# Mouafak-Khaled/Flow-Q-Learning

Hardware: AMD Instinct MI355X
Metric: FQL grad-steps/sec (whole node) over 16-α population, cube-single-v0 (higher is better)
Workload: dtype f32

## Files before the change

### flow-q-learning_amd/csrc/kernels.h

```cpp
#pragma once
#include <hip/hip_runtime.h>
#include <stdint.h>

namespace fq {

struct TRef {
    float* p;
    long long ss;
    long long sy;
};

inline TRef tref(float* p, long long ss, long long sy = 0) { return TRef{p, ss, sy}; }

enum GemmLayout { LAYOUT_FWD = 0, LAYOUT_DX = 1, LAYOUT_DW = 2 };
enum GemmEpi { EPI_STORE = 0, EPI_BIAS = 1, EPI_BIAS_GELU2 = 2, EPI_BIAS_GELU = 3, EPI_ADAM = 4 };

struct GemmArgs {
    TRef A, B, C, C2, bias;
    int M, N, K;
    int lda, ldb, ldc;
    int ny, nz;
    const int* slots;
    unsigned long long* probe;
};
void launch_gemm(int layout, int epi, int tile, const GemmArgs& a, hipStream_t s);
void launch_gemm_euler_hidden(const GemmArgs& a, hipStream_t s);
void launch_gemm_variant(int layout, int epi, int tile, int variant, const GemmArgs& a, hipStream_t s);
constexpr int GEMM_GROUP_MAX = 8;
constexpr int HP_COUNT = 3;
enum { HP_LR = 0, HP_DISCOUNT = 1, HP_TAU = 2 };
struct Chunk { long long off; int len; int leaf; };
struct AdamArgs {
    const float* p_in;
    float* p_out;
    float *g, *m, *v;
    float* target;
    long long P, PT;
    long long net_off;
    const Chunk* chunks;
    const int* ids;
    int n_chunks, chunk_base;
    float* stats;
    int n_total_chunks;
    const int* count;
    const float* hparams;
    int nz;
    const int* slots;
};
struct AdamEpi {
    const float* p_in;
    float *p_out, *m, *v, *target, *wt_out;
    long long P, PT, PTT;
    long long ens, wt_sy;
    long long w_off[GEMM_GROUP_MAX];
    long long wt_off[GEMM_GROUP_MAX];
    int stat_base[GEMM_GROUP_MAX];
    float* stats;
    int n_total_chunks;
    const int* count;
    const float* hparams;
    int mode;
    int nt;
    AdamArgs small;
    int small_blocks;
};
struct GemmGroupArgs {
    GemmArgs g[GEMM_GROUP_MAX];
    int first[GEMM_GROUP_MAX + 1];
    int ng;
    AdamEpi adam;
// ... 49 lines not shown
    long long w_off[EF_MAX_LAYERS + 1], b_off[EF_MAX_LAYERS + 1];
    long long g_off[EF_MAX_LAYERS], be_off[EF_MAX_LAYERS];
    const float* x0;
    long long x0_ss;
    int ld_x, K0, L, M;
    float* U[EF_MAX_LAYERS];
    float* G[EF_MAX_LAYERS];
    float* MU[EF_MAX_LAYERS];
    float* RS[EF_MAX_LAYERS];
    long long s_ss, s_sy, st_ss, st_sy;
    int ld_s, st_lo, st_hi;
    int g_hi;
    HeadArgs head;
    int ny, nz;
    const int* slots;
};
bool stream_fwd_supported(int H, int L, int K0, int nout, int M);
void launch_stream_fwd(int head_mode, bool ln, const StreamArgs& a, hipStream_t s);

struct SplitSync {
    unsigned long long* xch;
    unsigned* cnt;
    unsigned* gen;
    unsigned* err;
};
struct SplitFwdArgs {
    StreamArgs s;
    TRef aflow;
    int D, A, S, first;
    float steps_f;
// ... 303 lines not shown
```

### flow-q-learning_amd/csrc/kernels.hip

```cpp
#include "kernels.h"

#include <hip/hip_runtime.h>
#include <math.h>

#include <type_traits>

#if defined(__HIP_DEVICE_COMPILE__) && !defined(__gfx950__)
#error "fqlpop kernels target gfx950 (MI355X) only: the s_waitcnt immediates use the gfx9 encoding"
#endif


namespace fq {

typedef float f32x16 __attribute__((ext_vector_type(16)));
typedef float f32x4 __attribute__((ext_vector_type(4)));

#define DEV __device__ __forceinline__

DEV float* at(TRef t, int slot, int y = 0) {
    return t.p + (long long)slot * t.ss + (long long)y * t.sy;
}

constexpr float kSqrt2OverPi = 0.7978845608028654f;

// ... 106 lines not shown
    const int slot = a.slots[z];
    const Chunk ck = a.chunks[ci];
    const long long base = (long long)slot * a.P + a.net_off + ck.off;
    const float t = (float)(a.count[slot] + 1);
    const float bc1 = 1.0f - powf(0.9f, t), bc2 = 1.0f - powf(0.999f, t);
    float mx = -INFINITY, mn = INFINITY, ss = 0.f;
    const float* hp = a.hparams + (long long)slot * HP_COUNT;
    const float lr = hp[HP_LR], tau = hp[HP_TAU];
    const bool hasT = a.target != nullptr;
    if (NT == 256 || threadIdx.x < 256) {
        const float* __restrict__ Pin = a.p_in + base;
        float* __restrict__ P = a.p_out + base;
        const float* __restrict__ G = a.g + base;
        float* __restrict__ Mm = a.m + base;
        float* __restrict__ V = a.v + base;
        float* __restrict__ T = hasT ? a.target + (long long)slot * a.PT + ck.off : nullptr;
        auto one = [&](float g, float& p, float& m, float& v, float& tp) {
            adam_moments(g, m, v);
            if (hasT) tp = ema_target(p, tp, tau);
            p = adam_step_ieee(p, m, v, bc1, bc2, lr);
            mx = fmaxf(mx, g);
            mn = fminf(mn, g);
            ss = fmaf(g, g, ss);
        };
        if ((ck.len & 3) == 0) {
            for (int i = threadIdx.x * 4; i < ck.len; i += 1024) {
                const float4 g4 = *reinterpret_cast<const float4*>(G + i);
                float4 p4 = *reinterpret_cast<const float4*>(Pin + i);
                float4 m4 = *reinterpret_cast<float4*>(Mm + i);
                float4 v4 = *reinterpret_cast<float4*>(V + i);
                float4 t4 = make_float4(0.f, 0.f, 0.f, 0.f);
                if (hasT) t4 = *reinterpret_cast<float4*>(T + i);
                one(g4.x, p4.x, m4.x, v4.x, t4.x);
                one(g4.y, p4.y, m4.y, v4.y, t4.y);
                one(g4.z, p4.z, m4.z, v4.z, t4.z);
                one(g4.w, p4.w, m4.w, v4.w, t4.w);
                *reinterpret_cast<float4*>(P + i) = p4;
                *reinterpret_cast<float4*>(Mm + i) = m4;
                *reinterpret_cast<float4*>(V + i) = v4;
                if (hasT) *reinterpret_cast<float4*>(T + i) = t4;
            }
        } else {
            for (int i = threadIdx.x; i < ck.len; i += 256) {
                const float gv = G[i];
                float p = Pin[i], m = Mm[i], v = V[i], tv = hasT ? T[i] : 0.f;
                one(gv, p, m, v, tv);
                P[i] = p;
                Mm[i] = m;
                V[i] = v;
                if (hasT) T[i] = tv;
            }
        }
    }
    __shared__ float red[3 * 8];
    float st3[3] = {mx, mn, ss};
    block_reduce_n<3>(st3, {1, 2, 0}, red);
    mx = st3[0];
    mn = st3[1];
    ss = st3[2];
    if (threadIdx.x == 0) {
        float* st = a.stats + ((long long)slot * a.n_total_chunks + ci) * 3;
        st[0] = mx;
        st[1] = mn;
        st[2] = ss;
    }
// ... 98 lines not shown
    else __builtin_amdgcn_raw_buffer_store_b128(w, r, off_b, 0, 0);
}

constexpr int ADAM_U = 2;
struct AdamPre {
    float4 p[ADAM_U], m[ADAM_U], v[ADAM_U], t[ADAM_U];
};
template <int BM, int BN>
DEV void adam_issue0(const AdamEpi& e, int gi, const GemmArgs& g, int slot, int y, int i0, int j0, AdamPre& pre) {
    constexpr int TPR = BN / 4, RPI = 256 / TPR;
    const int gM = uni(g.M), ldc = uni(g.ldc), tid = threadIdx.x;
    const long long pb = uni64((long long)slot * e.P + e.w_off[gi] + (long long)y * e.ens);
    const long long nleaf = (long long)gM * ldc;
    const rsrc_t rP = make_rsrc(e.p_in + pb, nleaf);
    const rsrc_t rM = make_rsrc(e.m + pb, nleaf), rV = make_rsrc(e.v + pb, nleaf);
    const bool hasT = e.target != nullptr;
    const rsrc_t rT = make_rsrc(uniptr(hasT ? e.target + (long long)slot * e.PT + e.w_off[gi] + (long long)y * e.ens
                                            : e.m + pb), nleaf);
    const int cj = (tid % TPR) * 4, ri = tid / TPR;
#pragma unroll
    for (int u = 0; u < ADAM_U; ++u) {
        const int off = ((i0 + u * RPI + ri) * ldc + j0 + cj) * 4;
        pre.p[u] = bload4_aux(rP, off, 0);
        pre.m[u] = bload4_aux(rM, off, 1);
        pre.v[u] = bload4_aux(rV, off, 1);
        pre.t[u] = hasT ? bload4_aux(rT, off, 1) : float4{0.f, 0.f, 0.f, 0.f};
    }
}

template <int BM, int BN, bool DUAL, bool PRE>
DEV void adam_epilogue(const AdamEpi& e, int gi, const GemmArgs& g, f32x16 (&acc)[BM / 64][BN / 64],
                       f32x16 (&acc2)[BM / 64][BN / 64], int slot, int y, int tile, int per, int i0, int j0,
                       int wi, int wj, int l32, int lh, float* smem, const AdamPre& pre) {
    constexpr int TM = BM / 64, TN = BN / 64;
    constexpr int PT = BN + 1;
    const int gM = uni(g.M), ldc = uni(g.ldc), tid = threadIdx.x;
    const long long pb = uni64((long long)slot * e.P + e.w_off[gi] + (long long)y * e.ens);
    const long long nleaf = (long long)gM * ldc;
    const rsrc_t rP = make_rsrc(e.p_in + pb, nleaf), rPo = make_rsrc(e.p_out + pb, nleaf);
    const rsrc_t rM = make_rsrc(e.m + pb, nleaf), rV = make_rsrc(e.v + pb, nleaf);
    const bool hasT = e.target != nullptr;
    const rsrc_t rT = make_rsrc(uniptr(hasT ? e.target + (long long)slot * e.PT + e.w_off[gi] + (long long)y * e.ens
                                            : e.m + pb), nleaf);
    const float t = (float)(e.count[slot] + 1);
    const float bc1 = 1.0f - powf(0.9f, t), bc2 = 1.0f - powf(0.999f, t);
    const float rbc1 = 1.0f / bc1, rbc2 = 1.0f / bc2;
    const float* hp = e.hparams + (long long)slot * HP_COUNT;
    const float lr = uni_load(hp + HP_LR), tau = uni_load(hp + HP_TAU);
    float mx = -INFINITY, mn = INFINITY, ss = 0.f;
    const int rows = min(BM, gM - i0);
    const bool run = e.mode != 1;
    constexpr int TPR = BN / 4, RPI = 256 / TPR, U = ADAM_U, NB = BM / (RPI * U);
    static_assert(NB * RPI * U == BM && NB >= 2, "");
    const int cj = (tid % TPR) * 4, ri = tid / TPR;
    float4 p4[2][U], m4[2][U], v4[2][U], t4[2][U];
    auto issue = [&](int bi, int q) {
#pragma unroll
        for (int u = 0; u < U; ++u) {
// ... 44 lines not shown
                float tt[4] = {t4[q][u].x, t4[q][u].y, t4[q][u].z, t4[q][u].w};
#pragma unroll
                for (int c = 0; c < 4; ++c) {
                    const float gr = gs[c];
                    adam_moments(gr, mm[c], vv[c]);
                    tt[c] = ema_target(pp[c], tt[c], tau);
                    pp[c] = adam_step_fast(pp[c], mm[c], vv[c], rbc1, rbc2, lr);
                    gs[c] = pp[c];
                    mx = live ? fmaxf(mx, gr) : mx;
                    mn = live ? fminf(mn, gr) : mn;
                    ss = live ? fmaf(gr, gr, ss) : ss;
                }
                bstore4_aux(rPo, float4{pp[0], pp[1], pp[2], pp[3]}, off, 0);
                bstore4_aux(rM, float4{mm[0], mm[1], mm[2], mm[3]}, off, 1);
                bstore4_aux(rV, float4{vv[0], vv[1], vv[2], vv[3]}, off, 1);
                if (hasT) bstore4_aux(rT, float4{tt[0], tt[1], tt[2], tt[3]}, off, 1);
            }
        }
    }
    __shared__ float red[3 * 8];
    float st3[3] = {mx, mn, ss};
    block_reduce_n<3>(st3, {1, 2, 0}, red);
    mx = st3[0];
    mn = st3[1];
    ss = st3[2];
    if (tid == 0) {
        float* st = e.stats + ((long long)slot * e.n_total_chunks + e.stat_base[gi] + y * per + tile) * 3;
        st[0] = mx;
        st[1] = mn;
        st[2] = ss;
    }
// ... 843 lines not shown
#define FQ_HEAD_LAUNCH(KPT, MODE, grid, s, a) \
    hipLaunchKernelGGL((head_fwd_kernel<MODE, KPT>), grid, dim3(1024), 0, s, a)
void launch_head_fwd(int mode, const HeadArgs& a, hipStream_t s) {
    const dim3 grid((a.M / 64) * a.ny * a.nz);
    switch (mode) {
        case HEAD_STORE: FQ_KPT_DISPATCH(a.H, FQ_HEAD_LAUNCH, HEAD_STORE, grid, s, a) break;
        case HEAD_BC_FUSED: FQ_KPT_DISPATCH(a.H, FQ_HEAD_LAUNCH, HEAD_BC_FUSED, grid, s, a) break;
        case HEAD_EULER: FQ_KPT_DISPATCH(a.H, FQ_HEAD_LAUNCH, HEAD_EULER, grid, s, a) break;
        case HEAD_OS: FQ_KPT_DISPATCH(a.H, FQ_HEAD_LAUNCH, HEAD_OS, grid, s, a) break;
        default: FQ_KPT_DISPATCH(a.H, FQ_HEAD_LAUNCH, HEAD_ACT, grid, s, a) break;
    }
}

bool stream_fwd_supported(int H, int L, int K0, int nout, int M) {
    return H == EF_H && L >= 1 && L <= EF_MAX_LAYERS && K0 <= EF_K0MAX && nout <= 8 && M % EF_NC == 0;
}

template <int MODE, bool LN>
__global__ __launch_bounds__(EF_NW * 64, 1) void stream_fwd_kernel(const StreamArgs g) {
    constexpr int H = EF_H, NC = EF_NC, NT = EF_NW * 64, PF = EF_PF;
    __shared__ __attribute__((aligned(16))) float slab[H * NC + 64];
    __shared__ __attribute__((aligned(16))) float in0[EF_K0MAX * NC + 64];
    __shared__ float lnred[2][EF_NW][NC];
    __shared__ float lnp[3][H];

    const int tiles = g.M / NC;
    const int total = tiles * g.ny * g.nz;
    const int bid = xcd_remap(blockIdx.x, total);
    const int tile = bid % tiles, yz = bid / tiles;
    const int y = yz % g.ny, z = yz / g.ny;
// ... 3 lines not shown
    const int w = __builtin_amdgcn_readfirstlane(tid >> 6);
    const int li = lane & 15, lk = lane >> 4;
    const int L = g.L, K0 = g.K0, nout = g.head.nout;
    const bool tail0 = K0 > 4 * PF && K0 <= 4 * (PF + 1);
    const int NS0 = tail0 ? PF : (K0 + 4 * PF - 1) / (4 * PF) * PF;
    const float* __restrict__ P = g.params + (long long)slot * g.P + (long long)y * g.ens;
    const float* __restrict__ x0 = g.x0 + (long long)slot * g.x0_ss;
    load_in0<NT>(in0, x0, K0, g.ld_x, c0);
    const rsrc_t rW = make_rsrc(P, g.P);
    const int lo = lk * H + 64 * w + 4 * li;
    float4 ring[PF];
#pragma unroll
    for (int p = 0; p < PF; ++p) ring[p] = bload4(rW, (int)g.w_off[0] + 4 * p * H + lo);
    const bool st = c0 >= g.st_lo && c0 + NC <= g.st_hi;
    const int m = c0 + li;
    if constexpr (LN) {
        lnp[0][tid] = P[g.b_off[0] + tid];
        lnp[1][tid] = P[g.g_off[0] + tid];
        lnp[2][tid] = P[g.be_off[0] + tid];
    }
    __syncthreads();

    for (int l = 0; l < L; ++l) {
        const int NS = l == 0 ? NS0 : H / 4;
        const float* xs = l == 0 ? in0 : slab;
        const int nl = l + 1 < L ? l + 1 : 0;
        f32x4 acc[4];
#pragma unroll
        for (int c = 0; c < 4; ++c) acc[c] = f32x4{0.f, 0.f, 0.f, 0.f};
        const int lp = LN ? nl : l;
        const float pb = P[g.b_off[lp] + tid];
        const float pg = LN ? P[g.g_off[lp] + tid] : 0.f;
        const float pe = LN ? P[g.be_off[lp] + tid] : 0.f;
        const int wcur = (int)g.w_off[l], wnext = (int)g.w_off[nl];
        asm volatile("" ::"s"(wcur), "s"(wnext));
        const float4 at0 = bload4(rW, wcur + 4 * PF * H + lo);
        ef_kloop(acc, ring, rW, xs, NS, wcur, wnext, lo, lk, li);
        if (l == 0 && tail0) ef_tail(acc, at0, xs, lk, li);
        if constexpr (!LN) {
            lnp[0][tid] = pb;
            __syncthreads();
        }

        const bool stU = st && g.U[l], stG = st && g.G[l] && c0 + NC <= g.g_hi;
        const long long sbase = (long long)slot * g.s_ss + (long long)y * g.s_sy + c0;
        const rsrc_t rU = make_rsrc(stU ? g.U[l] + sbase : g.params, stU ? (long long)H * g.ld_s : 0);
        const rsrc_t rG = make_rsrc(stG ? g.G[l] + sbase : g.params, stG ? (long long)H * g.ld_s : 0);
        const int svo = ((64 * w + 16 * lk) * g.ld_s + li) * 4;
        float v[4][4];
// ... 2883 lines not shown
```

### flow-q-learning_amd/csrc/runtime.cpp

```cpp
#include <hip/hip_runtime.h>

#include <algorithm>
#include <cmath>
#include <cstdio>
#include <cstdlib>
#include <cstring>
#include <functional>
#include <map>
#include <set>
#include <memory>
#include <string>
#include <vector>

#include "../../include/fqlpop.h"
#include "kernels.h"
#include "popmem.h"

using namespace fq;

namespace {

constexpr long long kAlign = 64;
long long align_up(long long x) { return (x + kAlign - 1) / kAlign * kAlign; }

// ... 7 lines not shown
    int euler_fused = 1;
    int stream_fwd = 1;
    int stream_bwd = 1;
    int fused_adam = 1;
    int serial = 0;
    int dw_tile_critic = 10, dw_tile_actor = 10;
    int adam_nt = 3;
    int split = 1;
    int small_sched = 1;
    int split_blocks = 256;
    int split_sites = 0;
    int hw_queues = 4;
    int em_seq_sweep = 1;
    int em_ens_xcd = 0;
    int lazy_metric = 1;
};
EngineOptions g_engine_opts;

constexpr int kStepBranches = 4;
int step_streams(const EngineOptions& eo) {
    return (eo.serial || eo.hw_queues < kStepBranches) ? 1 : kStepBranches;
}

struct EngineOptionRef {
    const char* name;
    int EngineOptions::*field;
    int lo, hi;
};
const EngineOptionRef kEngineOptions[] = {
    {"euler_fused", &EngineOptions::euler_fused, 0, 1}, {"stream_fwd", &EngineOptions::stream_fwd, 0, 1},
    {"stream_bwd", &EngineOptions::stream_bwd, 0, 1},   {"fused_adam", &EngineOptions::fused_adam, 0, 1},
    {"serial", &EngineOptions::serial, 0, 1},
    {"dw_tile_critic", &EngineOptions::dw_tile_critic, 0, 10},
    {"dw_tile_actor", &EngineOptions::dw_tile_actor, 0, 10},
    {"adam_nt", &EngineOptions::adam_nt, 0, 3},
    {"split", &EngineOptions::split, 0, 8},
    {"small_sched", &EngineOptions::small_sched, 0, 1},
    {"hw_queues", &EngineOptions::hw_queues, 1, 1024},
    {"split_sites", &EngineOptions::split_sites, 0, (1 << 24) - 1},
    {"split_blocks", &EngineOptions::split_blocks, 64, 1024},
    {"em_seq_sweep", &EngineOptions::em_seq_sweep, 0, 1},
    {"em_ens_xcd", &EngineOptions::em_ens_xcd, 0, 1},
    {"lazy_metric", &EngineOptions::lazy_metric, 0, 1},
};

void philox_host(uint32_t c[4], uint32_t k0, uint32_t k1) {
    for (int r = 0; r < 10; ++r) {
        const uint64_t p0 = (uint64_t)0xD2511F53u * c[0], p1 = (uint64_t)0xCD9E8D57u * c[2];
        const uint32_t hi0 = (uint32_t)(p0 >> 32), lo0 = (uint32_t)p0;
        const uint32_t hi1 = (uint32_t)(p1 >> 32), lo1 = (uint32_t)p1;
        const uint32_t n0 = hi1 ^ c[1] ^ k0, n2 = hi0 ^ c[3] ^ k1;
        c[0] = n0; c[1] = lo1; c[2] = n2; c[3] = lo0;
        k0 += 0x9E3779B9u;
        k1 += 0xBB67AE85u;
    }
}

static_assert(HP_COUNT == FQLPOP_HP_COUNT && HP_LR == FQLPOP_HP_LR && HP_DISCOUNT == FQLPOP_HP_DISCOUNT &&
// ... 86 lines not shown
struct fqlpop : StepStreams<> {
    fqlpop_config cfg{};
    EngineOptions opt{};
    int n = 0;
    int device = 0;
    int D = 0, A = 0, H = 0, L = 0, B = 0, E = 0, S = 0;
    NetLayout critic, bc, os;
    long long P = 0, PT = 0;
    std::vector<Leaf> leaves;
    long long state_size = 0;

    DevBuf<float> params_buf[2];
    Buf paramsT_buf[2];
    int cur = 0;
    float *params = nullptr, *params_nx = nullptr;
    DevBuf<float> grads, adam_m, adam_v, target_buf;
    float* target = nullptr;
    DevBuf<int> count;
    DevBuf<uint64_t> seeds;
    DevBuf<uint64_t> skeys;
    DevBuf<float> alpha;
    DevBuf<float> hparams;
    DevBuf<int> slots;
    DevBuf<float> stats;
    DevBuf<Chunk> chunks;
    DevBuf<int> chunk_leaf;
    DevBuf<int> leaf_first;
    int n_chunks_net[3] = {0, 0, 0}, chunk_base_net[3] = {0, 0, 0}, n_chunks_total = 0;
    bool fused_adam = false;
    int w_stat_base[3][EF_MAX_LAYERS] = {};
    DevBuf<int> res_ids;
    int res_base[3] = {0, 0, 0}, res_n[3] = {0, 0, 0};
// ... 209 lines not shown
    for (size_t c = all_leaf.size(); c-- > 0;) first[all_leaf[c]] = (int)c;
    first[leaf_id] = (int)all_leaf.size();
    for (size_t c = 1; c < all_leaf.size(); ++c)
        ARGCHK(all_leaf[c] >= all_leaf[c - 1], "chunks of a leaf must be contiguous");
    h->leaf_first = DevBuf<int>(first.size(), "leaf chunk ranges");
    HIPCHK(hipMemcpy(h->leaf_first, first.data(), sizeof(int) * first.size(), hipMemcpyHostToDevice));
    h->chunk_leaf = DevBuf<int>(all_leaf.size(), "chunk leaves");
    HIPCHK(hipMemcpy(h->chunk_leaf, all_leaf.data(), sizeof(int) * all_leaf.size(), hipMemcpyHostToDevice));
    h->stats = DevBuf<float>(3 * all.size() * h->n, "gradient statistics");
    HIPCHK(hipMemset(h->stats, 0, sizeof(float) * 3 * all.size() * h->n));
}

void mirror_params(fqlpop* h, int slot, hipStream_t s) {
    HIPCHK(hipMemcpyAsync(h->params_nx + (long long)slot * h->P, h->params + (long long)slot * h->P,
                          sizeof(float) * h->P, hipMemcpyDeviceToDevice, s));
}

void upload_skey(fqlpop* h, int member) {
    const uint64_t k = sample_key(h->h_seeds[member], h->h_alpha[member]);
    HIPCHK(hipMemcpy(h->skeys + member, &k, sizeof(k), hipMemcpyHostToDevice));
}

void init_member(fqlpop* h, int slot, uint64_t seed) {
    unsigned salt = 1;
    auto init_net = [&](const NetLayout& N) {
        for (int e = 0; e < N.E; ++e) {
            float* base = h->params + (long long)slot * h->P + N.off + e * N.ens_size;
            for (int l = 0; l <= N.L; ++l) {
                const int fi = N.kdim(l), fo = N.ndim(l);
                InitArgs a{base + N.W[l], (long long)fi * fo, std::sqrt(6.0f / (float)(fi + fo)), 0.f, seed, salt++};
// ... 246 lines not shown
        gemm(LAYOUT_DW, EPI_STORE, gw, s);
        if (l > 0) {
            GemmArgs gx{};
            gx.A = n.par(N.W[l]);
            gx.B = n.grad(n.DU[l]);
            gx.C = n.grad(n.DH);
            gx.M = N.H; gx.N = k.M; gx.K = N.H;
            gx.lda = N.H; gx.ldb = n.ld_d; gx.ldc = n.ld_d;
            gx.ny = N.E; gx.nz = c.nz; gx.slots = h->slots;
            gemm(LAYOUT_DX, EPI_STORE, gx, s);
        }
    }
}

AdamArgs adam_args(const Ctx& c, int ni);
int skip_mask();

void stream_bwd_net(const Ctx& c, hipStream_t s, const Net& n, const BwdCols& k, TRef dout, hipStream_t sw,
                    const InGradArgs* ig = nullptr, std::function<void()>* defer = nullptr) {
    fqlpop* h = c.h;
    const NetLayout& N = *n.lay;
    const int M = k.M, Mg = k.Mg;
    StreamBwdArgs a{};
    a.params = *n.arena + N.off;
    a.P = n.arena_ss; a.ens = N.ens_size;
    a.paramsT = h->paramsT.p + h->wt_net_off[n.ni];
    a.PT = h->paramsT.ss; a.ensT = (long long)(N.L - 1) * N.H * N.H;
    for (int l = 1; l < N.L; ++l) a.wt_off[l] = (long long)(l - 1) * N.H * N.H;
    for (int l = 0; l <= N.L; ++l) {
        a.w_off[l] = N.W[l];
// ... 58 lines not shown
    for (int l = N.L - 1; l >= 0; --l) {
        GemmArgs gw{};
        gw.A = l == 0 ? n.X->cols(coff) : n.act(n.G[l - 1], coff);
        gw.B = n.grad(n.DU[l]);
        gw.C = pref(h, h->grads, N, N.W[l]);
        gw.M = N.kdim(l); gw.N = N.H; gw.K = Mg;
        gw.lda = n.ld; gw.ldb = n.ld_d; gw.ldc = N.H;
        gw.ny = N.E; gw.nz = c.nz; gw.slots = h->slots;
        gs.push_back(gw);
    }
    const int ni = n.ni;
    if (h->fused_adam) {
        AdamEpi ae{};
        ae.p_in = h->params; ae.p_out = h->params_nx; ae.m = h->adam_m; ae.v = h->adam_v;
        ae.target = ni == 0 ? h->target : nullptr;
        ae.wt_out = h->paramsT_nx.p;
        ae.P = h->P; ae.PT = h->PT; ae.PTT = h->paramsT_nx.ss;
        ae.ens = N.ens_size;
        ae.wt_sy = (long long)(N.L - 1) * N.H * N.H;
        for (int gi = 0; gi < (int)gs.size(); ++gi) {
            const int l = N.L - 1 - gi;
            ae.w_off[gi] = N.off + N.W[l];
            ae.wt_off[gi] = l >= 1 ? h->wt_net_off[ni] + (long long)(l - 1) * N.H * N.H : -1;
            ae.stat_base[gi] = h->w_stat_base[ni][l];
        }
        ae.stats = h->stats; ae.n_total_chunks = h->n_chunks_total;
        ae.count = h->count;
        ae.hparams = h->hparams;
        {
            const char* dm = diag_env("FQLPOP_DW_MODE");
            ae.mode = dm ? std::atoi(dm) : 0;
            if (ae.mode == 4) ae.mode = ni == 0 ? 0 : 3;
            ae.nt = h->opt.adam_nt;
        }
        ae.small = adam_args(c, ni);
        ae.small_blocks = ae.small.n_chunks * c.nz;
        launch_gemm_group_dw(dw_tile(h, N), gs.data(), (int)gs.size(), sw, &ae);
    } else if (N.L <= GEMM_GROUP_MAX && N.H % 128 == 0) {
// ... 26 lines not shown
            }
    }
    t.n_mats = n;
    if (all_slots) { t.slots = nullptr; t.nz = h->n; }
    else { t.slots = h->slots; t.nz = h->nz; }
    launch_transpose(t, s);
}

AdamArgs adam_args(const Ctx& c, int ni) {
    fqlpop* h = c.h;
    const NetLayout* nets[3] = {&h->critic, &h->bc, &h->os};
    AdamArgs a{};
    a.p_in = h->params; a.p_out = h->params_nx;
    a.g = h->grads; a.m = h->adam_m; a.v = h->adam_v;
    a.target = ni == 0 ? h->target : nullptr;
    a.P = h->P; a.PT = h->PT;
    a.net_off = nets[ni]->off;
    a.chunks = h->chunks;
    if (h->fused_adam) {
        a.ids = h->res_ids + h->res_base[ni];
        a.n_chunks = h->res_n[ni];
    } else {
        a.ids = nullptr;
        a.n_chunks = h->n_chunks_net[ni];
        a.chunk_base = h->chunk_base_net[ni];
    }
    a.stats = h->stats; a.n_total_chunks = h->n_chunks_total;
    a.count = h->count;
    a.hparams = h->hparams;
    a.nz = c.nz; a.slots = h->slots;
    return a;
}

void adam_net(const Ctx& c, hipStream_t s, int ni) {
    const AdamArgs a = adam_args(c, ni);
    if (a.n_chunks > 0) launch_adam(a, s);
}

struct FwdCols {
    int st_lo, st_hi;
    int g_hi = -1;
    int c0 = 0, M = -1;
};

void stream_fwd(const Ctx& c, hipStream_t s, const Net& n, const FwdCols& k, int mode, const HeadArgs& head) {
    fqlpop* h = c.h;
    const NetLayout& N = *n.lay;
    const bool store = k.st_hi > k.st_lo, stats = store && !n.MU.empty();
    const int M = k.M < 0 ? n.ld - k.c0 : k.M;
    ARGCHK(k.c0 % 16 == 0 && M > 0 && M % 16 == 0 && k.c0 + M <= n.ld && (!store || (k.c0 == 0 && k.st_hi <= M)),
           "streamed forward: bad column range");
    StreamArgs a{};
    a.params = *n.arena + N.off;
    a.P = n.arena_ss;
    a.ens = N.ens_size;
    for (int l = 0; l <= N.L; ++l) {
        a.w_off[l] = N.W[l];
        a.b_off[l] = N.b[l];
        if (l < N.L && N.ln) {
            a.g_off[l] = N.gam[l];
// ... 3 lines not shown
            a.U[l] = n.U[l].p;
            a.G[l] = n.G[l].p;
            if (stats && N.ln) { a.MU[l] = n.MU[l].p; a.RS[l] = n.RS[l].p; }
        }
    }
    a.x0 = n.X->p + k.c0;
    a.x0_ss = n.X->ss;
    a.ld_x = n.ld; a.K0 = N.in_dim; a.L = N.L; a.M = M;
    if (store) { a.s_ss = n.U[0].ss; a.s_sy = n.sy; }
    if (stats) { a.st_ss = n.MU[0].ss; a.st_sy = n.st_sy; }
    a.ld_s = n.ld; a.st_lo = k.st_lo; a.st_hi = k.st_hi;
    a.g_hi = k.g_hi < 0 ? k.st_hi : k.g_hi;
    a.head = head;
    a.head.nout = N.out_dim;
    a.ny = N.E; a.nz = c.nz; a.slots = h->slots;
    if (skip_mask() & n.skip_fwd) return;
    const int F = c.plan.F[n.fwd_site];
    if (F > 1) {
        SplitFwdArgs sa{};
        sa.s = a;
        sa.sync = split_prep(h, n.fwd_site, (long long)(M / 16) * N.E * c.nz, s);
        launch_split_fwd(mode, N.ln, false, F, sa, s);
    } else {
        launch_stream_fwd(mode, N.ln, a, s);
    }
}

long long euler_blocks(const Ctx& c) { return (long long)(c.h->B / 16) * c.nz * c.plan.F[SITE_EULER]; }
SplitFwdArgs euler_split_args(const Ctx& c, const EulerArgs& ea, hipStream_t s) {
    fqlpop* h = c.h;
// ... 206 lines not shown
    sa.tg_in = h->tg_in.ref();
    sa.eu_in = h->eu_in.ref();
    sa.act_t = h->act_t.ref();
    sa.x0_t = h->x0_t.ref();
    sa.rew_t = h->rew_t.ref();
    sa.mask_t = h->mask_t.ref();
    sa.nz = c.nz; sa.slots = h->slots;
    const bool lazy = train && h->lazy_metric;
    auto os_forward = [&]() {
        HeadArgs ha = head_args(c, h->n_os);
        ha.o0 = h->apiraw.ref(); ha.ld0 = B;
        ha.o1 = h->tg_in.ref(); ha.ld1 = B;
        ha.o2 = h->cr_in.ref(); ha.ld2 = B2;
        ha.o3 = h->amet.ref(); ha.ld3 = B;
        if (h->stream_fwd) {
            stream_fwd(c, sM, h->n_os, FwdCols{B, 2 * B, -1, 0, lazy ? B2 : 3 * B}, HEAD_OS, ha);
        } else {
            fwd_hidden(c, sM, h->n_os);
            launch_head_fwd(HEAD_OS, ha, sM);
        }
    };
    const bool ring = train && !inj_batch && h->synth.obs != nullptr;
    launch_sample(sa, sM, ring ? &h->synth : nullptr);
    HIPCHK(hipEventRecord(h->ev_sample, sM));
    if (sF != sM) HIPCHK(hipStreamWaitEvent(sF, h->ev_sample, 0));
    if (sB != sM) HIPCHK(hipStreamWaitEvent(sB, h->ev_sample, 0));

    LossArgs la{};
    la.q = h->q.ref(B2);
    la.qt = h->qt.ref(B);
    la.rew = h->rew_t.ref();
// ... 15 lines not shown
    la.info = (train ? h->info : h->vinfo).ref();
    la.metric = lazy ? 0 : 1;
    la.alpha = h->alpha;
    la.B = B; la.A = A; la.E = h->E;
    la.q_min = h->cfg.q_agg_min; la.normq = h->cfg.normalize_q_loss;
    la.hparams = h->hparams;
    la.nz = c.nz; la.slots = h->slots;

    {
        HeadArgs ha = head_args(c, h->n_bc);
        ha.o0 = h->vpred.ref(); ha.ld0 = B;
        ha.o1 = h->bc_in.ref(); ha.ld1 = B2;
        ha.o2 = h->eu_in.ref(); ha.ld2 = B;
        ha.t_next = (float)(1.0 / (double)S);
        if (h->stream_fwd) {
            stream_fwd(c, sF, h->n_bc, FwdCols{0, B}, HEAD_BC_FUSED, ha);
        } else {
            fwd_hidden(c, sF, h->n_bc);
            launch_head_fwd(HEAD_BC_FUSED, ha, sF);
        }
        HIPCHK(hipEventRecord(h->ev_bcfwd, sF));
        if (h->euler_fused) {
            EulerArgs ea = euler_args(h, c.nz);
            if (h->probe_set >= 0 && h->probe_idx < h->probe_pairs)
                ea.probe = h->probe_slots + 2 * h->probe_blocks * ((long long)h->probe_set * h->probe_pairs + h->probe_idx++);
            if (!(skip_mask() & h->n_eu.skip_fwd)) launch_euler(c, ea, sF);
        }
        for (int i = 1; !h->euler_fused && i < S + (S == 1 ? 1 : 0); ++i) {
            fwd_hidden(c, sF, h->n_eu);
            HeadArgs he = head_args(c, h->n_eu);
            he.o0 = h->aflow.ref(); he.ld0 = B;
// ... 15 lines not shown
        if (!h->fused_adam) {
            adam_net(c, sB, 1);
            if (h->stream_bwd) transpose_nets(h, sB, 2, false, h->params_nx, h->paramsT_nx);
        }
    }
    HIPCHK(hipEventRecord(h->ev_bdone, sB));

    os_forward();
    const bool small = c.plan.small;
    hipStream_t sT = small ? h->sX : sM;
    dep(sM, sT);
    if (h->stream_fwd) {
        HeadArgs ht{};
        ht.B = B; ht.D = D; ht.steps_f = (float)S;
        ht.o0 = h->qt.ref(B); ht.ld0 = B;
        stream_fwd(c, sT, h->n_tg, FwdCols{0, 0}, HEAD_STORE, ht);
    } else {
        fwd_hidden(c, sT, h->n_tg);
        HeadArgs ht = head_args(c, h->n_tg);
        ht.o0 = h->qt.ref(B); ht.ld0 = B;
        launch_head_fwd(HEAD_STORE, ht, sT);
    }
    {
        HeadArgs hc = head_args(c, h->n_cr);
        hc.o0 = h->q.ref(B2); hc.ld0 = B2;
        if (h->stream_fwd) {
            stream_fwd(c, sM, h->n_cr, FwdCols{0, B2, h->stream_bwd ? B : B2}, HEAD_STORE, hc);
        } else {
            fwd_hidden(c, sM, h->n_cr);
            launch_head_fwd(HEAD_STORE, hc, sM);
        }
    }
    dep(sT, sM);
    launch_loss_critic(la, sM);
    std::function<void()> critic_dw;
    if (train) {
        const Net& cr = h->n_cr;
        InGradArgs ig{};
        ig.W0 = cr.par(h->critic.W[0]);
        ig.du0 = cr.grad(cr.DU[0]);
        ig.da = h->da.ref();
        ig.H = h->H; ig.D = D; ig.A = A; ig.E = h->E; ig.ld = B2; ig.off = B; ig.M = B;
// ... 43 lines not shown
        fa.count = h->count;
        fa.nz = c.nz; fa.slots = h->slots;
        launch_finalize(fa, sM);
    } else if (sB != sM) {
        HIPCHK(hipStreamWaitEvent(sM, h->ev_bdone, 0));
    }
    HIPCHK(hipGetLastError());
}

void flip_params(fqlpop* h) {
    h->cur ^= 1;
    h->params = h->params_buf[h->cur];
    h->params_nx = h->params_buf[h->cur ^ 1];
    h->paramsT = h->paramsT_buf[h->cur];
    h->paramsT_nx = h->paramsT_buf[h->cur ^ 1];
}

Graphs& graph_for(fqlpop* h, bool train, bool inj_batch, bool inj_noise, bool recapture);

void drop_graphs(fqlpop* h) { h->graphs.clear(); }

void clear_metric_tail(fqlpop* h) {
    fqlpop::SplitSite& st = h->split_site[SITE_OSF];
    if (!h->lazy_metric || !st.xch || split_plan(h, h->nz).F[SITE_OSF] <= 1) return;
    const long long third = (long long)(h->B / 16) * h->nz, words = split_cluster_bytes() / 8;
    unsigned long long* x = st.xch;
    HIPCHK(hipMemsetAsync(x + 2 * third * words, 0, split_cluster_bytes() * third, h->sM));
}

void run(fqlpop* h, bool train, bool inj_batch, bool inj_noise) {
// ... 293 lines not shown
        h->bc.off = align_up(h->critic.size());
        h->os.off = align_up(h->bc.off + h->bc.size());
        h->P = align_up(h->os.off + h->os.size());
        h->PT = align_up(h->critic.size());
        build_leaves(h.get());

        h->opt = g_engine_opts;
        const EngineOptions& eo = h->opt;
        h->make_streams(step_streams(eo));
        h->ev_pool.resize(64);
        h->euler_fused = euler_flow_supported(H, L, D, A, B) && !h->bc.ln && eo.euler_fused;
        h->stream_fwd = stream_fwd_supported(H, L, D + A + 1, A, B) && eo.stream_fwd;
        h->stream_bwd = stream_bwd_supported(H, L, A, B, B) && eo.stream_bwd;
        h->lazy_metric = h->stream_fwd && eo.lazy_metric;
        h->fused_adam = h->stream_bwd && H % 128 == 0 && L <= GEMM_GROUP_MAX && h->critic.off == 0 && eo.fused_adam;
        if (h->euler_fused) {
            h->probe_pairs = 1;
            h->probe_blocks = std::max<long long>((long long)(cfg->batch_size / 16) * n_members * 8, kSplitMaxBlocks);
        } else {
            h->probe_pairs = std::max(1, (cfg->flow_steps - 1) * (cfg->num_hidden - 1));
            h->probe_blocks = (long long)((cfg->hidden_dim + 63) / 64) * ((cfg->batch_size + 63) / 64) * n_members;
        }
        const size_t pb = sizeof(unsigned long long) * 4 * h->probe_blocks * h->probe_pairs;
        constexpr unsigned kMapped = hipHostMallocMapped | hipHostMallocCoherent;
        using Stamps = HostBuf<unsigned long long>;
        h->probe_host = Stamps(4 * h->probe_blocks * h->probe_pairs, kMapped, "probe stamps");
#ifdef FQ_PHASE_PROBE
        if (const char* e = diag_env("FQLPOP_PHASE_PROBE"); e != nullptr && e[0] == '1') {
            h->phase_blocks = (long long)(2 * cfg->batch_size / 16) * E * n_members;
            const size_t phb = sizeof(unsigned long long) * SB_PHASE_STRIDE * h->phase_blocks;
// ... 18 lines not shown
            *e = Event<>(hipEventDisableTiming);
        h->ev_t0 = Event<>(hipEventDefault);
        h->ev_t1 = Event<>(hipEventDefault);

        const int n = h->n;
        const size_t Pn = (size_t)h->P * n;
        for (auto& pb : h->params_buf) {
            pb = DevBuf<float>(Pn, "parameters");
            HIPCHK(hipMemset(pb, 0, sizeof(float) * Pn));
        }
        h->params = h->params_buf[0];
        h->params_nx = h->params_buf[1];
        h->grads = DevBuf<float>(Pn, "gradients");
        h->adam_m = DevBuf<float>(Pn, "Adam first moments");
        h->adam_v = DevBuf<float>(Pn, "Adam second moments");
        h->target_buf = DevBuf<float>((size_t)h->PT * n, "target critic");
        h->target = h->target_buf;
        HIPCHK(hipMemset(h->grads, 0, sizeof(float) * Pn));
        h->count = DevBuf<int>(n, "step counts");
        h->seeds = DevBuf<uint64_t>(n, "member seeds");
        h->skeys = DevBuf<uint64_t>(n, "sampler keys");
        h->alpha = DevBuf<float>(n, "member alphas");
        h->hparams = DevBuf<float>((size_t)n * FQLPOP_HP_COUNT, "member hparams");
        h->slots = DevBuf<int>(n, "active slots");
        build_chunks(h.get());

        const int Kc = D + A, Kb = D + A + 1, B2 = 2 * B, B3 = 3 * B;
        auto input = [&](int K, int ld) { return h->alloc(align_up((long long)K * ld), (long long)K * ld); };
        h->os_in = input(Kc, B3);
        h->bc_in = input(Kb, B2);
        h->eu_in = input(Kb, B);
        for (Buf& cb : h->cr_in_buf) cb = input(Kc, B2);
// ... 489 lines not shown
                throw Err{FQLPOP_E_STATE, "member " + std::to_string(src[i]) + "'s state was written by a failed "
                                            "split launch; restore it before cloning from it"};
        CloneArgs base{};
        auto arena = [&](const float* s, const float* s_idle, float* d, long long stride) {
            if (stride <= 0 || d == nullptr) return;
            ARGCHK(base.n_arenas < CLONE_MAX_ARENAS && stride % 4 == 0, "clone arena table");
            base.arena[base.n_arenas++] = CloneArena{s, s_idle, d, stride, stride / 4};
        };
        arena(h->params, h->params, h->params, h->P);
        arena(h->params_nx, h->params, h->params_nx, h->P);
        if (h->stream_bwd) {
            arena(h->paramsT.p, h->paramsT.p, h->paramsT.p, h->paramsT.ss);
            arena(h->paramsT_nx.p, h->paramsT.p, h->paramsT_nx.p, h->paramsT_nx.ss);
        }
        arena(h->target, h->target, h->target, h->PT);
        arena(h->adam_m, h->adam_m, h->adam_m, h->P);
        arena(h->adam_v, h->adam_v, h->adam_v, h->P);
        base.count = h->count; base.alpha = h->alpha; base.hparams = h->hparams; base.seed = h->seeds; base.skey = h->skeys;
        for (int p0 = 0; p0 < n_pairs; p0 += CLONE_MAX_PAIRS) {
            CloneArgs a = base;
            a.n_pairs = std::min(CLONE_MAX_PAIRS, n_pairs - p0);
            for (int i = 0; i < a.n_pairs; ++i) {
                a.src[i] = src[p0 + i]; a.dst[i] = dst[p0 + i];
                a.dst_idle[i] = h->active[dst[p0 + i]] ? 0 : 1;
                a.alphas[i] = alphas[p0 + i]; a.seeds[i] = seeds[p0 + i];
                a.skeys[i] = sample_key(seeds[p0 + i], alphas[p0 + i]);
            }
            launch_clone(a, h->sM);
            if (h->synth.obs) {
                SynthCloneArgs sc{};
// ... 789 lines not shown
```

Baseline: 8475.

## Move transposed-weight copies and target EMA into streaming forward kernels

Adds a copy path inside the streaming forward kernel. While a layer's weights are streamed, spare tiles either write the transposed weight copy (using permlane swaps) or compute the target-network EMA and write it to a new double-buffered target array. The fused Adam epilogue then skips those writes for the layers the forward already handled. The aim is to take these weight-sized read/write passes off the critical backward/Adam epilogue and hide them under forward compute. In exchange it doubles target memory, adds an extra copy in mirror/clone, and adds per-layer work to the forward kernels.

```diff
diff --git a/flow-q-learning_amd/csrc/kernels.h b/flow-q-learning_amd/csrc/kernels.h
--- a/flow-q-learning_amd/csrc/kernels.h
+++ b/flow-q-learning_amd/csrc/kernels.h
@@ -34,7 +34,8 @@
     const float* p_in;
     float* p_out;
     float *g, *m, *v;
-    float* target;
+    const float* target;
+    float* target_out;
     long long P, PT;
     long long net_off;
     const Chunk* chunks;
@@ -48,12 +49,13 @@
     const int* slots;
 };
 struct AdamEpi {
-    const float* p_in;
-    float *p_out, *m, *v, *target, *wt_out;
+    const float *p_in, *target;
+    float *p_out, *m, *v, *target_out, *wt_out;
     long long P, PT, PTT;
     long long ens, wt_sy;
     long long w_off[GEMM_GROUP_MAX];
     long long wt_off[GEMM_GROUP_MAX];
+    int no_ema[GEMM_GROUP_MAX];
     int stat_base[GEMM_GROUP_MAX];
     float* stats;
     int n_total_chunks;
@@ -133,6 +135,12 @@
     HeadArgs head;
     int ny, nz;
     const int* slots;
+    float* wt_out;
+    long long wt_ss, wt_sy;
+    float* ema_out;
+    const float* ema_src;
+    long long ema_ss;
+    const float* hparams;
 };
 bool stream_fwd_supported(int H, int L, int K0, int nout, int M);
 void launch_stream_fwd(int head_mode, bool ln, const StreamArgs& a, hipStream_t s);
diff --git a/flow-q-learning_amd/csrc/kernels.hip b/flow-q-learning_amd/csrc/kernels.hip
--- a/flow-q-learning_amd/csrc/kernels.hip
+++ b/flow-q-learning_amd/csrc/kernels.hip
@@ -144,7 +144,8 @@
         const float* __restrict__ G = a.g + base;
         float* __restrict__ Mm = a.m + base;
         float* __restrict__ V = a.v + base;
-        float* __restrict__ T = hasT ? a.target + (long long)slot * a.PT + ck.off : nullptr;
+        const float* __restrict__ T = hasT ? a.target + (long long)slot * a.PT + ck.off : nullptr;
+        float* __restrict__ To = hasT ? a.target_out + (long long)slot * a.PT + ck.off : nullptr;
         auto one = [&](float g, float& p, float& m, float& v, float& tp) {
             adam_moments(g, m, v);
             if (hasT) tp = ema_target(p, tp, tau);
@@ -160,7 +161,7 @@
                 float4 m4 = *reinterpret_cast<float4*>(Mm + i);
                 float4 v4 = *reinterpret_cast<float4*>(V + i);
                 float4 t4 = make_float4(0.f, 0.f, 0.f, 0.f);
-                if (hasT) t4 = *reinterpret_cast<float4*>(T + i);
+                if (hasT) t4 = *reinterpret_cast<const float4*>(T + i);
                 one(g4.x, p4.x, m4.x, v4.x, t4.x);
                 one(g4.y, p4.y, m4.y, v4.y, t4.y);
                 one(g4.z, p4.z, m4.z, v4.z, t4.z);
@@ -168,7 +169,7 @@
                 *reinterpret_cast<float4*>(P + i) = p4;
                 *reinterpret_cast<float4*>(Mm + i) = m4;
                 *reinterpret_cast<float4*>(V + i) = v4;
-                if (hasT) *reinterpret_cast<float4*>(T + i) = t4;
+                if (hasT) *reinterpret_cast<float4*>(To + i) = t4;
             }
         } else {
             for (int i = threadIdx.x; i < ck.len; i += 256) {
@@ -178,7 +179,7 @@
                 P[i] = p;
                 Mm[i] = m;
                 V[i] = v;
-                if (hasT) T[i] = tv;
+                if (hasT) To[i] = tv;
             }
         }
     }
@@ -307,7 +308,7 @@
     const long long nleaf = (long long)gM * ldc;
     const rsrc_t rP = make_rsrc(e.p_in + pb, nleaf);
     const rsrc_t rM = make_rsrc(e.m + pb, nleaf), rV = make_rsrc(e.v + pb, nleaf);
-    const bool hasT = e.target != nullptr;
+    const bool hasT = e.target != nullptr && !uni(e.no_ema[gi]);
     const rsrc_t rT = make_rsrc(uniptr(hasT ? e.target + (long long)slot * e.PT + e.w_off[gi] + (long long)y * e.ens
                                             : e.m + pb), nleaf);
     const int cj = (tid % TPR) * 4, ri = tid / TPR;
@@ -332,9 +333,10 @@
     const long long nleaf = (long long)gM * ldc;
     const rsrc_t rP = make_rsrc(e.p_in + pb, nleaf), rPo = make_rsrc(e.p_out + pb, nleaf);
     const rsrc_t rM = make_rsrc(e.m + pb, nleaf), rV = make_rsrc(e.v + pb, nleaf);
-    const bool hasT = e.target != nullptr;
-    const rsrc_t rT = make_rsrc(uniptr(hasT ? e.target + (long long)slot * e.PT + e.w_off[gi] + (long long)y * e.ens
-                                            : e.m + pb), nleaf);
+    const bool hasT = e.target != nullptr && !uni(e.no_ema[gi]);
+    const long long tb = uni64((long long)slot * e.PT + e.w_off[gi] + (long long)y * e.ens);
+    const rsrc_t rT = make_rsrc(uniptr(hasT ? e.target + tb : e.m + pb), nleaf);
+    const rsrc_t rTo = make_rsrc(uniptr(hasT ? e.target_out + tb : e.m + pb), nleaf);
     const float t = (float)(e.count[slot] + 1);
     const float bc1 = 1.0f - powf(0.9f, t), bc2 = 1.0f - powf(0.999f, t);
     const float rbc1 = 1.0f / bc1, rbc2 = 1.0f / bc2;
@@ -409,7 +411,7 @@
                 bstore4_aux(rPo, float4{pp[0], pp[1], pp[2], pp[3]}, off, 0);
                 bstore4_aux(rM, float4{mm[0], mm[1], mm[2], mm[3]}, off, 1);
                 bstore4_aux(rV, float4{vv[0], vv[1], vv[2], vv[3]}, off, 1);
-                if (hasT) bstore4_aux(rT, float4{tt[0], tt[1], tt[2], tt[3]}, off, 1);
+                if (hasT) bstore4_aux(rTo, float4{tt[0], tt[1], tt[2], tt[3]}, off, 1);
             }
         }
     }
@@ -1283,6 +1285,55 @@
 
 bool stream_fwd_supported(int H, int L, int K0, int nout, int M) {
     return H == EF_H && L >= 1 && L <= EF_MAX_LAYERS && K0 <= EF_K0MAX && nout <= 8 && M % EF_NC == 0;
+}
+
+DEV void lk_transpose(float4& a) {
+    asm volatile("s_nop 1\n\tv_permlane16_swap_b32 %0, %1" : "+v"(a.x), "+v"(a.y));
+    asm volatile("s_nop 1\n\tv_permlane16_swap_b32 %0, %1" : "+v"(a.z), "+v"(a.w));
+    asm volatile("s_nop 1\n\tv_permlane32_swap_b32 %0, %1" : "+v"(a.x), "+v"(a.z));
+    asm volatile("s_nop 1\n\tv_permlane32_swap_b32 %0, %1" : "+v"(a.y), "+v"(a.w));
+}
+
+DEV void fwd_copies(const StreamArgs& g, rsrc_t rW, int wcur, int lo, int l, int tile, int own, int slot, int y,
+                    int w, int lk, int li) {
+    constexpr int H = EF_H;
+    const bool ema = g.ema_out != nullptr;
+    const long long mo = (long long)slot * g.P + (long long)y * g.ens;
+    const rsrc_t rO = ema ? make_rsrc(g.ema_out + mo, g.ens)
+                          : make_rsrc(g.wt_out + (long long)slot * g.wt_ss + (long long)y * g.wt_sy +
+                                          (long long)(l - 1) * H * H, (long long)H * H);
+    const rsrc_t rC = make_rsrc(ema ? g.ema_src + (long long)slot * g.ema_ss + (long long)y * g.ens : g.params, ema ? g.ens : 0);
+    const float tau = ema ? uni_load(g.hparams + (long long)slot * HP_COUNT + HP_TAU) : 0.f;
+    int lo_ = lo;
+    asm volatile("" : "+v"(lo_));
+    const int to = ((lo_ & (H - 1)) + lo_ / H) * H;
+    constexpr int CH = 1;
+#pragma unroll 1
+    for (int q = tile; q < H / 32; q += own) {
+#pragma unroll 1
+        for (int s0 = 8 * q; s0 < 8 * q + 8; s0 += CH) {
+            float4 a[CH], c[CH];
+#pragma unroll
+            for (int p = 0; p < CH; ++p) a[p] = bload4(rW, wcur + 4 * (s0 + p) * H + lo);
+            if (ema) {
+#pragma unroll
+                for (int p = 0; p < CH; ++p) c[p] = bload4(rC, wcur + 4 * (s0 + p) * H + lo);
+#pragma unroll
+                for (int p = 0; p < CH; ++p) {
+                    const float4 t = a[p];
+                    const float4 r{ema_target(c[p].x, t.x, tau), ema_target(c[p].y, t.y, tau),
+                                   ema_target(c[p].z, t.z, tau), ema_target(c[p].w, t.w, tau)};
+                    bstore4_aux(rO, r, (wcur + 4 * (s0 + p) * H + lo) * 4, 0);
+                }
+            } else {
+#pragma unroll
+                for (int p = 0; p < CH; ++p) {
+                    lk_transpose(a[p]);
+                    bstore4_aux(rO, a[p], (to + 4 * (s0 + p)) * 4, 0);
+                }
+            }
+        }
+    }
 }
 
 template <int MODE, bool LN>
@@ -1316,6 +1367,8 @@
     for (int p = 0; p < PF; ++p) ring[p] = bload4(rW, (int)g.w_off[0] + 4 * p * H + lo);
     const bool st = c0 >= g.st_lo && c0 + NC <= g.st_hi;
     const int m = c0 + li;
+    const bool copies = g.wt_out != nullptr || g.ema_out != nullptr;
+    const int own = tiles < H / 32 ? tiles : H / 32;
     if constexpr (LN) {
         lnp[0][tid] = P[g.b_off[0] + tid];
         lnp[1][tid] = P[g.g_off[0] + tid];
@@ -1335,6 +1388,7 @@
         const float pg = LN ? P[g.g_off[lp] + tid] : 0.f;
         const float pe = LN ? P[g.be_off[lp] + tid] : 0.f;
         const int wcur = (int)g.w_off[l], wnext = (int)g.w_off[nl];
+        if (l >= 1 && copies && tile < own) fwd_copies(g, rW, wcur, lo, l, tile, own, slot, y, w, lk, li);
         asm volatile("" ::"s"(wcur), "s"(wnext));
         const float4 at0 = bload4(rW, wcur + 4 * PF * H + lo);
         ef_kloop(acc, ring, rW, xs, NS, wcur, wnext, lo, lk, li);
diff --git a/flow-q-learning_amd/csrc/runtime.cpp b/flow-q-learning_amd/csrc/runtime.cpp
--- a/flow-q-learning_amd/csrc/runtime.cpp
+++ b/flow-q-learning_amd/csrc/runtime.cpp
@@ -45,6 +45,7 @@
     int em_seq_sweep = 1;
     int em_ens_xcd = 0;
     int lazy_metric = 1;
+    int fwd_copies = 2;
 };
 EngineOptions g_engine_opts;
 
@@ -73,6 +74,7 @@
     {"em_seq_sweep", &EngineOptions::em_seq_sweep, 0, 1},
     {"em_ens_xcd", &EngineOptions::em_ens_xcd, 0, 1},
     {"lazy_metric", &EngineOptions::lazy_metric, 0, 1},
+    {"fwd_copies", &EngineOptions::fwd_copies, 0, 3},
 };
 
 void philox_host(uint32_t c[4], uint32_t k0, uint32_t k1) {
@@ -189,8 +191,9 @@
     Buf paramsT_buf[2];
     int cur = 0;
     float *params = nullptr, *params_nx = nullptr;
-    DevBuf<float> grads, adam_m, adam_v, target_buf;
-    float* target = nullptr;
+    DevBuf<float> grads, adam_m, adam_v, target_buf[2];
+    float *target = nullptr, *target_nx = nullptr;
+    int fwd_copies = 0;
     DevBuf<int> count;
     DevBuf<uint64_t> seeds;
     DevBuf<uint64_t> skeys;
@@ -430,6 +433,8 @@
 void mirror_params(fqlpop* h, int slot, hipStream_t s) {
     HIPCHK(hipMemcpyAsync(h->params_nx + (long long)slot * h->P, h->params + (long long)slot * h->P,
                           sizeof(float) * h->P, hipMemcpyDeviceToDevice, s));
+    HIPCHK(hipMemcpyAsync(h->target_nx + (long long)slot * h->PT, h->target + (long long)slot * h->PT,
+                          sizeof(float) * h->PT, hipMemcpyDeviceToDevice, s));
 }
 
 void upload_skey(fqlpop* h, int member) {
@@ -706,6 +711,7 @@
 }
 
 AdamArgs adam_args(const Ctx& c, int ni);
+bool fwd_writes(const Ctx& c, const Net& n, int bit);
 int skip_mask();
 
 void stream_bwd_net(const Ctx& c, hipStream_t s, const Net& n, const BwdCols& k, TRef dout, hipStream_t sw,
@@ -794,14 +800,18 @@
         AdamEpi ae{};
         ae.p_in = h->params; ae.p_out = h->params_nx; ae.m = h->adam_m; ae.v = h->adam_v;
         ae.target = ni == 0 ? h->target : nullptr;
+        ae.target_out = h->target_nx;
         ae.wt_out = h->paramsT_nx.p;
+        const bool ema_fwd = ni == 0 && fwd_writes(c, h->n_tg, 2);
+        const bool wt_fwd = fwd_writes(c, ni == 0 ? h->n_cr : ni == 1 ? h->n_bc : h->n_os, 1);
         ae.P = h->P; ae.PT = h->PT; ae.PTT = h->paramsT_nx.ss;
         ae.ens = N.ens_size;
         ae.wt_sy = (long long)(N.L - 1) * N.H * N.H;
         for (int gi = 0; gi < (int)gs.size(); ++gi) {
             const int l = N.L - 1 - gi;
             ae.w_off[gi] = N.off + N.W[l];
-            ae.wt_off[gi] = l >= 1 ? h->wt_net_off[ni] + (long long)(l - 1) * N.H * N.H : -1;
+            ae.wt_off[gi] = l >= 1 && !wt_fwd ? h->wt_net_off[ni] + (long long)(l - 1) * N.H * N.H : -1;
+            ae.no_ema[gi] = l >= 1 && ema_fwd ? 1 : 0;
             ae.stat_base[gi] = h->w_stat_base[ni][l];
         }
         ae.stats = h->stats; ae.n_total_chunks = h->n_chunks_total;
@@ -858,6 +868,7 @@
     a.p_in = h->params; a.p_out = h->params_nx;
     a.g = h->grads; a.m = h->adam_m; a.v = h->adam_v;
     a.target = ni == 0 ? h->target : nullptr;
+    a.target_out = h->target_nx;
     a.P = h->P; a.PT = h->PT;
     a.net_off = nets[ni]->off;
     a.chunks = h->chunks;
@@ -881,13 +892,18 @@
     if (a.n_chunks > 0) launch_adam(a, s);
 }
 
+bool fwd_writes(const Ctx& c, const Net& n, int bit) {
+    return (c.h->fwd_copies & bit) != 0 && n.lay->L > 1 && c.plan.F[n.fwd_site] <= 1;
+}
+
 struct FwdCols {
     int st_lo, st_hi;
     int g_hi = -1;
     int c0 = 0, M = -1;
 };
 
-void stream_fwd(const Ctx& c, hipStream_t s, const Net& n, const FwdCols& k, int mode, const HeadArgs& head) {
+void stream_fwd(const Ctx& c, hipStream_t s, const Net& n, const FwdCols& k, int mode, const HeadArgs& head,
+                bool copies = false) {
     fqlpop* h = c.h;
     const NetLayout& N = *n.lay;
     const bool store = k.st_hi > k.st_lo, stats = store && !n.MU.empty();
@@ -921,6 +937,16 @@
     a.head = head;
     a.head.nout = N.out_dim;
     a.ny = N.E; a.nz = c.nz; a.slots = h->slots;
+    if (copies && n.arena == &h->target) {
+        if (fwd_writes(c, n, 2)) {
+            a.ema_out = h->target_nx + N.off;
+            a.ema_src = h->params + N.off; a.ema_ss = h->P;
+            a.hparams = h->hparams;
+        }
+    } else if (copies && fwd_writes(c, n, 1)) {
+        a.wt_out = h->paramsT.p + h->wt_net_off[n.ni];
+        a.wt_ss = h->paramsT.ss; a.wt_sy = (long long)(N.L - 1) * N.H * N.H;
+    }
     if (skip_mask() & n.skip_fwd) return;
     const int F = c.plan.F[n.fwd_site];
     if (F > 1) {
@@ -1157,7 +1183,7 @@
         ha.o2 = h->cr_in.ref(); ha.ld2 = B2;
         ha.o3 = h->amet.ref(); ha.ld3 = B;
         if (h->stream_fwd) {
-            stream_fwd(c, sM, h->n_os, FwdCols{B, 2 * B, -1, 0, lazy ? B2 : 3 * B}, HEAD_OS, ha);
+            stream_fwd(c, sM, h->n_os, FwdCols{B, 2 * B, -1, 0, lazy ? B2 : 3 * B}, HEAD_OS, ha, train);
         } else {
             fwd_hidden(c, sM, h->n_os);
             launch_head_fwd(HEAD_OS, ha, sM);
@@ -1203,7 +1229,7 @@
         ha.o2 = h->eu_in.ref(); ha.ld2 = B;
         ha.t_next = (float)(1.0 / (double)S);
         if (h->stream_fwd) {
-            stream_fwd(c, sF, h->n_bc, FwdCols{0, B}, HEAD_BC_FUSED, ha);
+            stream_fwd(c, sF, h->n_bc, FwdCols{0, B}, HEAD_BC_FUSED, ha, train);
         } else {
             fwd_hidden(c, sF, h->n_bc);
             launch_head_fwd(HEAD_BC_FUSED, ha, sF);
@@ -1249,7 +1275,7 @@
         HeadArgs ht{};
         ht.B = B; ht.D = D; ht.steps_f = (float)S;
         ht.o0 = h->qt.ref(B); ht.ld0 = B;
-        stream_fwd(c, sT, h->n_tg, FwdCols{0, 0}, HEAD_STORE, ht);
+        stream_fwd(c, sT, h->n_tg, FwdCols{0, 0}, HEAD_STORE, ht, train);
     } else {
         fwd_hidden(c, sT, h->n_tg);
         HeadArgs ht = head_args(c, h->n_tg);
@@ -1260,7 +1286,7 @@
         HeadArgs hc = head_args(c, h->n_cr);
         hc.o0 = h->q.ref(B2); hc.ld0 = B2;
         if (h->stream_fwd) {
-            stream_fwd(c, sM, h->n_cr, FwdCols{0, B2, h->stream_bwd ? B : B2}, HEAD_STORE, hc);
+            stream_fwd(c, sM, h->n_cr, FwdCols{0, B2, h->stream_bwd ? B : B2}, HEAD_STORE, hc, train);
         } else {
             fwd_hidden(c, sM, h->n_cr);
             launch_head_fwd(HEAD_STORE, hc, sM);
@@ -1334,6 +1360,8 @@
     h->params_nx = h->params_buf[h->cur ^ 1];
     h->paramsT = h->paramsT_buf[h->cur];
     h->paramsT_nx = h->paramsT_buf[h->cur ^ 1];
+    h->target = h->target_buf[h->cur];
+    h->target_nx = h->target_buf[h->cur ^ 1];
 }
 
 Graphs& graph_for(fqlpop* h, bool train, bool inj_batch, bool inj_noise, bool recapture);
@@ -1657,6 +1685,7 @@
         h->stream_bwd = stream_bwd_supported(H, L, A, B, B) && eo.stream_bwd;
         h->lazy_metric = h->stream_fwd && eo.lazy_metric;
         h->fused_adam = h->stream_bwd && H % 128 == 0 && L <= GEMM_GROUP_MAX && h->critic.off == 0 && eo.fused_adam;
+        h->fwd_copies = h->stream_fwd && h->fused_adam ? eo.fwd_copies : 0;
         if (h->euler_fused) {
             h->probe_pairs = 1;
             h->probe_blocks = std::max<long long>((long long)(cfg->batch_size / 16) * n_members * 8, kSplitMaxBlocks);
@@ -1705,8 +1734,9 @@
         h->grads = DevBuf<float>(Pn, "gradients");
         h->adam_m = DevBuf<float>(Pn, "Adam first moments");
         h->adam_v = DevBuf<float>(Pn, "Adam second moments");
-        h->target_buf = DevBuf<float>((size_t)h->PT * n, "target critic");
-        h->target = h->target_buf;
+        for (auto& tb : h->target_buf) tb = DevBuf<float>((size_t)h->PT * n, "target critic");
+        h->target = h->target_buf[0];
+        h->target_nx = h->target_buf[1];
         HIPCHK(hipMemset(h->grads, 0, sizeof(float) * Pn));
         h->count = DevBuf<int>(n, "step counts");
         h->seeds = DevBuf<uint64_t>(n, "member seeds");
@@ -2226,6 +2256,7 @@
             arena(h->paramsT_nx.p, h->paramsT.p, h->paramsT_nx.p, h->paramsT_nx.ss);
         }
         arena(h->target, h->target, h->target, h->PT);
+        arena(h->target_nx, h->target, h->target_nx, h->PT);
         arena(h->adam_m, h->adam_m, h->adam_m, h->P);
         arena(h->adam_v, h->adam_v, h->adam_v, h->P);
         base.count = h->count; base.alpha = h->alpha; base.hparams = h->hparams; base.seed = h->seeds; base.skey = h->skeys;
```

Measured after the change: 8624 (median of 6 runs). 1.8% higher.
